# ISU-PAAL/DeepDFA

Hardware: NVIDIA H100
Metric: CFG graphs/sec (train step) (higher is better)
Workload: dtype f32 (GRU GEMMs: bf16x3 split operands, f32 accumulate)

## Files before the change

deepdfa_b200/csrc/gru_tc_fwd3.cu:

```cuda
#include <cuda_fp16.h>
#include <stdlib.h>

#include "tc_common.cuh"

namespace ddfa {
namespace tc3 {
using namespace tcc;

constexpr int kSlices = 4;
constexpr int kSliceCols = kD / kSlices;
constexpr int kRowsPerPart = 3 * kSliceCols;
constexpr int kWChunkBytes = kRowsPerPart * 128;
constexpr int kSliceWBytes = 8 * kWChunkBytes;
constexpr int kStageBytes = kImageTileBytes;
constexpr int kOffStage = kSliceWBytes;
constexpr int kOffBias = kOffStage + 2 * kStageBytes;
constexpr int kBiasSlice = 7 * kSliceCols;
constexpr int kOffBar = kOffBias + kBiasSlice * 4;
constexpr int kSmemAlloc = kOffBar + 5 * 8;
constexpr int kConsumerWarps = 8;
constexpr int kThreads = 32 * kConsumerWarps + 32;
constexpr size_t kPackedWBytes = (size_t)kSlices * kSliceWBytes;
constexpr size_t kPackedBytes = kPackedWBytes + (size_t)kSlices * kBiasSlice * 4;
static_assert(kSmemAlloc <= 232448, "shared memory budget");

__global__ void pack_kernel(const float *__restrict__ w_fold, const float *__restrict__ w_hh, const float *__restrict__ b_fold,
                            const float *__restrict__ b_ih, const float *__restrict__ b_hh, uint8_t *__restrict__ packed) {
  const int idx = blockIdx.x * blockDim.x + threadIdx.x;
  if (idx >= kSlices * 2 * kRowsPerPart * 16) return;
  const int u = idx % 16, n = (idx / 16) % kRowsPerPart, p = (idx / (16 * kRowsPerPart)) % 2, slice = idx / (32 * kRowsPerPart);
  const int kb = u >> 3, k0 = u * 8;
  const float *W = (p == 0 ? w_fold : w_hh) + (size_t)((n / kSliceCols) * kD + slice * kSliceCols + n % kSliceCols) * kD;
  float x[8];
#pragma unroll
  for (int i = 0; i < 8; ++i) x[i] = W[k0 + i];
  uint4 ph, pl;
  split8(x, ph, pl);
  uint8_t *base = packed + (size_t)slice * kSliceWBytes + sw128_offset(n, (u & 7) * 8);
  *reinterpret_cast<uint4 *>(base + ((p * 2 + 0) * 2 + kb) * kWChunkBytes) = ph;
  *reinterpret_cast<uint4 *>(base + ((p * 2 + 1) * 2 + kb) * kWChunkBytes) = pl;
  if (p == 0 && u == 0 && n < kSliceCols) {
    const int t = slice * kSliceCols + n;
    float *bias = reinterpret_cast<float *>(packed + kPackedWBytes) + slice * kBiasSlice;
    bias[0 * kSliceCols + n] = b_ih[2 * kD + t];
    bias[1 * kSliceCols + n] = b_ih[t] + b_hh[t];
    bias[2 * kSliceCols + n] = b_ih[kD + t] + b_hh[kD + t];
    bias[3 * kSliceCols + n] = b_hh[2 * kD + t];
    bias[4 * kSliceCols + n] = b_fold[2 * kD + t];
    bias[5 * kSliceCols + n] = b_fold[t];
    bias[6 * kSliceCols + n] = b_fold[kD + t];
  }
}

template <bool HIMG, int GATES>
__global__ void __launch_bounds__(kThreads, 1) gru_fwd3_kernel(const uint8_t *__restrict__ s_img, const uint8_t *__restrict__ h_img,
                                                               const float *__restrict__ h, const int32_t *__restrict__ indptr,
                                                               const uint8_t *__restrict__ packed, int32_t N,
                                                               float *__restrict__ h_out, uint8_t *__restrict__ h_out_img,
                                                               float *__restrict__ gates, uint2 *__restrict__ gates_packed, int hints) {
  extern __shared__ __align__(1024) uint8_t smem[];
  const uint32_t sbase = smem_u32(smem);
  if ((sbase & 1023u) != 0) __trap();
  const uint32_t bar0 = sbase + kOffBar;
  auto full = [&](int i) { return bar0 + 8u * i; };
  auto empty = [&](int i) { return bar0 + 8u * (2 + i); };
  const uint32_t w_full = bar0 + 32u;

  const int warp = threadIdx.x >> 5, lane = threadIdx.x & 31;
  const int slice = blockIdx.x % kSlices;
  const int group = blockIdx.x / kSlices, num_groups = gridDim.x / kSlices;
  const int num_tiles = (N + kTileM - 1) / kTileM;
  const int my_tiles = (num_tiles > group) ? (num_tiles - 1 - group) / num_groups + 1 : 0;

  if (threadIdx.x == 0) {
    for (int i = 0; i < 2; ++i) { mbar_init(full(i), 1); mbar_init(empty(i), kConsumerWarps); }
    mbar_init(w_full, 1);
    mbar_fence_init();
  }
  __syncthreads();
  const int tron = g_trace_on;
  if (threadIdx.x == 0) trace_stamp(tron, 0, 0);
  pdl_launch_dependents();

  if (warp == kConsumerWarps) {
    if (my_tiles > 0 && elect_one()) {
      mbar_arrive_expect_tx(w_full, kSliceWBytes);
      bulk_g2s(sbase, packed + (size_t)slice * kSliceWBytes, kSliceWBytes, w_full);
      pdl_wait();
      for (int k = 0; k < my_tiles; ++k) {
        const size_t toff = (size_t)(group + k * num_groups) * kImageTileBytes;
        for (int p = 0; p < 2; ++p) {
          if (k > 0) mbar_wait_bounded(empty(p), (k - 1) & 1);
          mbar_arrive_expect_tx(full(p), kStageBytes);
          bulk_g2s(sbase + kOffStage + p * kStageBytes, (p == 0 ? s_img : h_img) + toff, kStageBytes, full(p));
          trace_stamp(tron, k, 1 + p);
        }
      }
    }
    return;
  }

  float *sbias = reinterpret_cast<float *>(smem + kOffBias);
  for (int i = threadIdx.x; i < kBiasSlice; i += 32 * kConsumerWarps)
    sbias[i] = __ldcg(reinterpret_cast<const float *>(packed + kPackedWBytes) + slice * kBiasSlice + i);
  asm volatile("bar.sync 1, %0;" ::"n"(32 * kConsumerWarps) : "memory");
  pdl_wait();
  if (my_tiles == 0) return;
  const int wg = warp >> 2;
  const int row0 = wg * 64 + (warp & 3) * 16 + (lane >> 2);
  const int c4 = 2 * (lane & 3);
  const size_t plane = (size_t)N * kD;
  const uint64_t pol_gates = l2_policy((hints & 1) ? 1 : 0);
  const uint64_t pol_next = l2_policy((hints & 16) ? 2 : 0);
  mbar_wait_bounded(w_full, 0);
  const bool tr = (warp == 0 && lane == 0);

  for (int k = 0; k < my_tiles; ++k) {
    const int tile = group + k * num_groups;
    float acc_s[48], acc_h[48];
    if (tr) { trace_stamp(tron, k, 7); trace_stamp(tron, k, 3); }
    mbar_wait_bounded(full(0), k & 1);
    if (tr) trace_stamp(tron, k, 4);
    wgmma_fence();
#pragma unroll
    for (int p = 0; p < 2; ++p) {
      if (p == 1) {
        mbar_wait_bounded(full(1), k & 1);
        if (tr) trace_stamp(tron, k, 5);
      }
      const uint32_t a0 = sbase + kOffStage + p * kStageBytes + wg * 8192;
      const uint32_t w0 = sbase + p * 4 * kWChunkBytes;
#pragma unroll
      for (int kb = 0; kb < 2; ++kb) {
#pragma unroll
        for (int k4 = 0; k4 < 4; ++k4) {
          const uint64_t a_hi = gmma_desc(a0 + kb * kChunkBytes + k4 * 32), a_lo = gmma_desc(a0 + (2 + kb) * kChunkBytes + k4 * 32);
          const uint64_t b_hi = gmma_desc(w0 + kb * kWChunkBytes + k4 * 32), b_lo = gmma_desc(w0 + (2 + kb) * kWChunkBytes + k4 * 32);
          const uint32_t acc = (kb == 0 && k4 == 0) ? 0u : 1u;
          if (p == 0) {
            wgmma_n96<0, 0>(acc_s, a_hi, b_hi, acc);
            wgmma_n96<0, 0>(acc_s, a_hi, b_lo, 1u);
            wgmma_n96<0, 0>(acc_s, a_lo, b_hi, 1u);
          } else {
            wgmma_n96<0, 0>(acc_h, a_hi, b_hi, acc);
            wgmma_n96<0, 0>(acc_h, a_hi, b_lo, 1u);
            wgmma_n96<0, 0>(acc_h, a_lo, b_hi, 1u);
          }
        }
      }
      wgmma_commit();
    }
    float deg[2], hp[2][8];
#pragma unroll
    for (int hh = 0; hh < 2; ++hh) {
      const int64_t node = (int64_t)tile * kTileM + row0 + 8 * hh;
      const bool valid = node < N;
      deg[hh] = valid ? (float)(__ldcg(indptr + node + 1) - __ldcg(indptr + node)) : 0.f;
#pragma unroll
      for (int j = 0; j < 4; ++j) {
        const int gcol = slice * kSliceCols + 8 * j + c4;
        if constexpr (HIMG) {
          const uint32_t whi = __ldcg(reinterpret_cast<const uint32_t *>(h_img + image_offset(node, gcol, 0)));
          const uint32_t wlo = __ldcg(reinterpret_cast<const uint32_t *>(h_img + image_offset(node, gcol, 1)));
          hp[hh][2 * j] = __uint_as_float(whi << 16) + __uint_as_float(wlo << 16);
          hp[hh][2 * j + 1] = __uint_as_float(whi & 0xffff0000u) + __uint_as_float(wlo & 0xffff0000u);
        } else {
          const float2 v = valid ? __ldcg(reinterpret_cast<const float2 *>(h + node * kD + gcol)) : make_float2(0.f, 0.f);
          hp[hh][2 * j] = v.x;
          hp[hh][2 * j + 1] = v.y;
        }
      }
    }
    wgmma_wait<0>();
    wgmma_fence_regs(acc_s);
    wgmma_fence_regs(acc_h);
    if (tr) { trace_stamp(tron, k, 6); trace_stamp(tron, k, 8); }
    __syncwarp();
    if (lane == 0) { mbar_arrive(empty(0)); mbar_arrive(empty(1)); }
    if (tr) trace_stamp(tron, k, 9);

#pragma unroll
    for (int hh = 0; hh < 2; ++hh) {
      const int64_t node = (int64_t)tile * kTileM + row0 + 8 * hh;
      const bool valid = node < N;
#pragma unroll
      for (int j = 0; j < 4; ++j) {
        const int c = 8 * j + c4, gcol = slice * kSliceCols + c;
        float hn[2], rr[2], zz[2], nn[2], gg[2];
#pragma unroll
        for (int e = 0; e < 2; ++e) {
          const int i = 2 * hh + e;
          const float dg = deg[hh];
          const float gin = acc_s[4 * (8 + j) + i] + fmaf(dg, sbias[4 * kSliceCols + c + e], sbias[c + e]);
          const float r = fast_sigmoid(acc_s[4 * j + i] + acc_h[4 * j + i] + fmaf(dg, sbias[5 * kSliceCols + c + e], sbias[kSliceCols + c + e]));
          const float z = fast_sigmoid(acc_s[4 * (4 + j) + i] + acc_h[4 * (4 + j) + i] +
                                       fmaf(dg, sbias[6 * kSliceCols + c + e], sbias[2 * kSliceCols + c + e]));
          const float ghn = acc_h[4 * (8 + j) + i] + sbias[3 * kSliceCols + c + e];
          const float n = fast_tanh(fmaf(r, ghn, gin));
          hn[e] = valid ? fmaf(z, hp[hh][2 * j + e] - n, n) : 0.f;
          rr[e] = r; zz[e] = z; nn[e] = n; gg[e] = ghn;
        }
        const size_t off = (size_t)node * kD + gcol;
        if (valid && h_out != nullptr) st_f2_hint(h_out + off, make_float2(hn[0], hn[1]), pol_next);
        if constexpr (GATES == 2) {
          if (valid) {
            const uint2 g0 = pack_gates(rr[0], zz[0], nn[0], gg[0]), g1 = pack_gates(rr[1], zz[1], nn[1], gg[1]);
            st_u4_hint(gates_packed + off, make_uint4(g0.x, g0.y, g1.x, g1.y), pol_gates);
          }
        }
        if constexpr (GATES == 1) {
          if (valid) {
            st_f2_hint(gates + off, make_float2(rr[0], rr[1]), pol_gates);
            st_f2_hint(gates + plane + off, make_float2(zz[0], zz[1]), pol_gates);
            st_f2_hint(gates + 2 * plane + off, make_float2(nn[0], nn[1]), pol_gates);
            st_f2_hint(gates + 3 * plane + off, make_float2(gg[0], gg[1]), pol_gates);
          }
        }
        if (h_out_img != nullptr) {
          const uint32_t hw = bf16x2_bits(hn[0], hn[1]);
          const uint32_t lw = bf16x2_bits(hn[0] - __uint_as_float(hw << 16), hn[1] - __uint_as_float(hw & 0xffff0000u));
          st_u32_hint(h_out_img + image_offset(node, gcol, 0), hw, pol_next);
          st_u32_hint(h_out_img + image_offset(node, gcol, 1), lw, pol_next);
        }
      }
    }
    if (tr) trace_stamp(tron, k, 10);
  }
}

}

size_t gru_tc3_packed_bytes() { return tc3::kPackedBytes; }

int gru_tc3_prepare(const float *w_fold, const float *b_fold, const float *b_ih, const float *w_hh, const float *b_hh, void *packed,
                    cudaStream_t stream) {
  const int total = tc3::kSlices * 2 * tc3::kRowsPerPart * 16;
  tc3::pack_kernel<<<(total + 127) / 128, 128, 0, stream>>>(w_fold, w_hh, b_fold, b_ih, b_hh, static_cast<uint8_t *>(packed));
  DDFA_CHECK_LAUNCH("tc3::pack_kernel");
  chain_break();
  return DDFA_OK;
}

int gru_tc3_step_fwd(const void *s_img, const void *h_img, const float *h, const int32_t *indptr, int32_t N, float *h_out,
                     void *h_out_img, float *save_gates, void *save_gates_packed, const void *packed, cudaStream_t stream) {
  const int tiles = (N + tcc::kTileM - 1) / tcc::kTileM;
  int groups = kNumSMs / tc3::kSlices;
  if (groups > tiles) groups = tiles;
  if (save_gates && save_gates_packed) {
    set_error("tcgen05 engine (fwd): both gate formats requested");
    return DDFA_ERR_INVALID_ARG;
  }
  if ((h == nullptr && save_gates) ) {
    set_error("tcgen05 engine (fwd): fp32 gate planes go with the fp32 h operand (legacy form)");
    return DDFA_ERR_INVALID_ARG;
  }
  if (tiles == 0) return DDFA_OK;
#define DDFA_FWD3_LAUNCH(HIMG, GATES)                                                                                                     \
  do {                                                                                                                                   \
    DDFA_CUDA(cudaFuncSetAttribute(tc3::gru_fwd3_kernel<HIMG, GATES>, cudaFuncAttributeMaxDynamicSharedMemorySize, tc3::kSmemAlloc));     \
    DDFA_CUDA(launch_chain(2, tc3::gru_fwd3_kernel<HIMG, GATES>, dim3(groups * tc3::kSlices), dim3(tc3::kThreads), tc3::kSmemAlloc,        \
                           stream, static_cast<const uint8_t *>(s_img), static_cast<const uint8_t *>(h_img), h, indptr,                   \
                           static_cast<const uint8_t *>(packed), N, h_out, static_cast<uint8_t *>(h_out_img), save_gates,                \
                           static_cast<uint2 *>(save_gates_packed), l2_hints()));                                                        \
  } while (0)
  if (h) {
    if (save_gates) DDFA_FWD3_LAUNCH(false, 1);
    else if (save_gates_packed) DDFA_FWD3_LAUNCH(false, 2);
    else DDFA_FWD3_LAUNCH(false, 0);
  } else {
    if (save_gates_packed) DDFA_FWD3_LAUNCH(true, 2);
    else DDFA_FWD3_LAUNCH(true, 0);
  }
#undef DDFA_FWD3_LAUNCH
  DDFA_CHECK_LAUNCH("tc3::gru_fwd3_kernel");
  return DDFA_OK;
}

namespace tc3 {
__global__ void __launch_bounds__(256) to_image_kernel(const float *__restrict__ x, int32_t N, uint8_t *__restrict__ image) {
  const int64_t t = blockIdx.x * (int64_t)blockDim.x + threadIdx.x;
  const int64_t rows = ((int64_t)N + kTileM - 1) / kTileM * kTileM;
  if (t >= rows * 16) return;
  const int64_t node = t >> 4;
  const int col = (int)(t & 15) * 8;
  float v[8] = {0.f, 0.f, 0.f, 0.f, 0.f, 0.f, 0.f, 0.f};
  if (node < N) {
    const float4 a = ldg_nc_f4(x + node * kD + col), b = ldg_nc_f4(x + node * kD + col + 4);
    v[0] = a.x; v[1] = a.y; v[2] = a.z; v[3] = a.w; v[4] = b.x; v[5] = b.y; v[6] = b.z; v[7] = b.w;
  }
  uint4 ph, pl;
  split8(v, ph, pl);
  *reinterpret_cast<uint4 *>(image + image_offset(node, col, 0)) = ph;
  *reinterpret_cast<uint4 *>(image + image_offset(node, col, 1)) = pl;
}
}

size_t act_image_bytes(int64_t n) { return tcc::image_bytes(n); }

int act_to_image(const float *x, int32_t N, void *image, cudaStream_t stream) {
  const int64_t rows = ((int64_t)N + tcc::kTileM - 1) / tcc::kTileM * tcc::kTileM;
  const int64_t total = rows * 16;
  if (total == 0) return DDFA_OK;
  tc3::to_image_kernel<<<(unsigned)((total + 255) / 256), 256, 0, stream>>>(x, N, static_cast<uint8_t *>(image));
  DDFA_CHECK_LAUNCH("to_image_kernel");
  return DDFA_OK;
}

size_t gru_tc2_workspace_bytes() { return gru_tc3_packed_bytes(); }

int gru_tc2_prepare(const float *w_fold, const float *b_fold, const float *b_ih, const float *w_hh, const float *b_hh,
                    void *workspace, size_t workspace_bytes, cudaStream_t stream) {
  if (workspace == nullptr || workspace_bytes < gru_tc2_workspace_bytes()) {
    set_error("tcgen05 engine: workspace too small (%zu < %zu)", workspace_bytes, gru_tc2_workspace_bytes());
    return DDFA_ERR_WORKSPACE;
  }
  return gru_tc3_prepare(w_fold, b_fold, b_ih, w_hh, b_hh, workspace, stream);
}

int gru_tc2_step_fwd(const void *s_img, const void *h_img, const float *h, const int32_t *indptr, int32_t N, float *h_out,
                     void *h_out_img, float *save_gates, void *save_gates_packed, const void *workspace, size_t workspace_bytes,
                     cudaStream_t stream) {
  if (workspace == nullptr || workspace_bytes < gru_tc2_workspace_bytes()) {
    set_error("tcgen05 engine: workspace too small (%zu < %zu)", workspace_bytes, gru_tc2_workspace_bytes());
    return DDFA_ERR_WORKSPACE;
  }
  return gru_tc3_step_fwd(s_img, h_img, h, indptr, N, h_out, h_out_img, save_gates, save_gates_packed, workspace, stream);
}

int gru_tc3_trace_enable(int on) {
  DDFA_CUDA(cudaMemcpyToSymbol(tcc::g_trace_on, &on, sizeof(int)));
  return DDFA_OK;
}
int gru_tc3_trace_read(void *host, size_t bytes) {
  if (bytes > tcc::kTraceWords * sizeof(long long)) bytes = tcc::kTraceWords * sizeof(long long);
  DDFA_CUDA(cudaMemcpyFromSymbol(host, tcc::g_trace, bytes));
  return DDFA_OK;
}

}
```

Before: 115,200.

## Split stage barriers per warpgroup and ping-pong wgmma issue between warpgroups

Each stage load is split into per-warpgroup halves, each with its own full/empty mbarriers, so a warpgroup can start as soon as its own 64 rows have arrived. The two consumer warpgroups take turns issuing their wgmma sequences via named barriers (bar.sync/bar.arrive), so one warpgroup's GEMM can overlap the other's epilogue. It also interleaves the s and h GEMMs inside the k loop. The cost is more bulk copies (four chunk copies per half), extra barrier traffic, and serialized MMA issue, which could leave the tensor cores idle if the epilogues are short.

Result: no change. 115,500 (median of 6 runs) (+0.3%).

```diff
diff --git a/deepdfa_b200/csrc/gru_tc_fwd3.cu b/deepdfa_b200/csrc/gru_tc_fwd3.cu
--- a/deepdfa_b200/csrc/gru_tc_fwd3.cu
+++ b/deepdfa_b200/csrc/gru_tc_fwd3.cu
@@ -17,9 +17,12 @@
 constexpr int kOffBias = kOffStage + 2 * kStageBytes;
 constexpr int kBiasSlice = 7 * kSliceCols;
 constexpr int kOffBar = kOffBias + kBiasSlice * 4;
-constexpr int kSmemAlloc = kOffBar + 5 * 8;
+constexpr int kSmemAlloc = kOffBar + 9 * 8;
 constexpr int kConsumerWarps = 8;
 constexpr int kThreads = 32 * kConsumerWarps + 32;
+constexpr int kHalfRowsBytes = 64 * 128;
+constexpr int kHalfStageBytes = 4 * kHalfRowsBytes;
+constexpr int kTurn0 = 2, kTurn1 = 3;
 constexpr size_t kPackedWBytes = (size_t)kSlices * kSliceWBytes;
 constexpr size_t kPackedBytes = kPackedWBytes + (size_t)kSlices * kBiasSlice * 4;
 static_assert(kSmemAlloc <= 232448, "shared memory budget");
@@ -62,9 +65,9 @@
   const uint32_t sbase = smem_u32(smem);
   if ((sbase & 1023u) != 0) __trap();
   const uint32_t bar0 = sbase + kOffBar;
-  auto full = [&](int i) { return bar0 + 8u * i; };
-  auto empty = [&](int i) { return bar0 + 8u * (2 + i); };
-  const uint32_t w_full = bar0 + 32u;
+  auto full = [&](int p, int wg) { return bar0 + 8u * (2 * p + wg); };
+  auto empty = [&](int p, int wg) { return bar0 + 8u * (4 + 2 * p + wg); };
+  const uint32_t w_full = bar0 + 64u;
 
   const int warp = threadIdx.x >> 5, lane = threadIdx.x & 31;
   const int slice = blockIdx.x % kSlices;
@@ -73,7 +76,8 @@
   const int my_tiles = (num_tiles > group) ? (num_tiles - 1 - group) / num_groups + 1 : 0;
 
   if (threadIdx.x == 0) {
-    for (int i = 0; i < 2; ++i) { mbar_init(full(i), 1); mbar_init(empty(i), kConsumerWarps); }
+    for (int p = 0; p < 2; ++p)
+      for (int wg = 0; wg < 2; ++wg) { mbar_init(full(p, wg), 1); mbar_init(empty(p, wg), kConsumerWarps / 2); }
     mbar_init(w_full, 1);
     mbar_fence_init();
   }
@@ -89,11 +93,16 @@
       pdl_wait();
       for (int k = 0; k < my_tiles; ++k) {
         const size_t toff = (size_t)(group + k * num_groups) * kImageTileBytes;
-        for (int p = 0; p < 2; ++p) {
-          if (k > 0) mbar_wait_bounded(empty(p), (k - 1) & 1);
-          mbar_arrive_expect_tx(full(p), kStageBytes);
-          bulk_g2s(sbase + kOffStage + p * kStageBytes, (p == 0 ? s_img : h_img) + toff, kStageBytes, full(p));
-          trace_stamp(tron, k, 1 + p);
+        for (int wg = 0; wg < 2; ++wg) {
+          for (int p = 0; p < 2; ++p) {
+            if (k > 0) mbar_wait_bounded(empty(p, wg), (k - 1) & 1);
+            mbar_arrive_expect_tx(full(p, wg), kHalfStageBytes);
+            const uint32_t dst = sbase + kOffStage + p * kStageBytes + wg * kHalfRowsBytes;
+            const uint8_t *src = (p == 0 ? s_img : h_img) + toff + wg * kHalfRowsBytes;
+#pragma unroll
+            for (int c = 0; c < 4; ++c) bulk_g2s(dst + c * kChunkBytes, src + c * kChunkBytes, kHalfRowsBytes, full(p, wg));
+          }
+          trace_stamp(tron, k, 1 + wg);
         }
       }
     }
@@ -114,42 +123,48 @@
   const uint64_t pol_next = l2_policy((hints & 16) ? 2 : 0);
   mbar_wait_bounded(w_full, 0);
   const bool tr = (warp == 0 && lane == 0);
+  const bool tr1 = (warp == 4 && lane == 0);
+  auto wait_turn = [&]() {
+    if (wg == 0) asm volatile("bar.sync %0, %1;" ::"n"(kTurn0), "n"(32 * kConsumerWarps) : "memory");
+    else asm volatile("bar.sync %0, %1;" ::"n"(kTurn1), "n"(32 * kConsumerWarps) : "memory");
+  };
+  auto pass_turn = [&]() {
+    if (wg == 0) asm volatile("bar.arrive %0, %1;" ::"n"(kTurn1), "n"(32 * kConsumerWarps) : "memory");
+    else asm volatile("bar.arrive %0, %1;" ::"n"(kTurn0), "n"(32 * kConsumerWarps) : "memory");
+  };
 
   for (int k = 0; k < my_tiles; ++k) {
     const int tile = group + k * num_groups;
     float acc_s[48], acc_h[48];
-    if (tr) { trace_stamp(tron, k, 7); trace_stamp(tron, k, 3); }
-    mbar_wait_bounded(full(0), k & 1);
+    if (tr) trace_stamp(tron, k, 7);
+    if (wg == 1 || k > 0) wait_turn();
+    if (tr) trace_stamp(tron, k, 3);
+    mbar_wait_bounded(full(0, wg), k & 1);
     if (tr) trace_stamp(tron, k, 4);
+    mbar_wait_bounded(full(1, wg), k & 1);
+    if (tr) trace_stamp(tron, k, 5);
     wgmma_fence();
-#pragma unroll
-    for (int p = 0; p < 2; ++p) {
-      if (p == 1) {
-        mbar_wait_bounded(full(1), k & 1);
-        if (tr) trace_stamp(tron, k, 5);
+    const uint32_t a0 = sbase + kOffStage + wg * kHalfRowsBytes;
+#pragma unroll
+    for (int kb = 0; kb < 2; ++kb) {
+#pragma unroll
+      for (int k4 = 0; k4 < 4; ++k4) {
+        const uint32_t acc = (kb == 0 && k4 == 0) ? 0u : 1u;
+#pragma unroll
+        for (int p = 0; p < 2; ++p) {
+          const uint32_t ap = a0 + p * kStageBytes, wp = sbase + p * 4 * kWChunkBytes;
+          const uint64_t a_hi = gmma_desc(ap + kb * kChunkBytes + k4 * 32), a_lo = gmma_desc(ap + (2 + kb) * kChunkBytes + k4 * 32);
+          const uint64_t b_hi = gmma_desc(wp + kb * kWChunkBytes + k4 * 32), b_lo = gmma_desc(wp + (2 + kb) * kWChunkBytes + k4 * 32);
+          float(&d)[48] = p == 0 ? acc_s : acc_h;
+          wgmma_n96<0, 0>(d, a_hi, b_hi, acc);
+          wgmma_n96<0, 0>(d, a_hi, b_lo, 1u);
+          wgmma_n96<0, 0>(d, a_lo, b_hi, 1u);
+        }
       }
-      const uint32_t a0 = sbase + kOffStage + p * kStageBytes + wg * 8192;
-      const uint32_t w0 = sbase + p * 4 * kWChunkBytes;
-#pragma unroll
-      for (int kb = 0; kb < 2; ++kb) {
-#pragma unroll
-        for (int k4 = 0; k4 < 4; ++k4) {
-          const uint64_t a_hi = gmma_desc(a0 + kb * kChunkBytes + k4 * 32), a_lo = gmma_desc(a0 + (2 + kb) * kChunkBytes + k4 * 32);
-          const uint64_t b_hi = gmma_desc(w0 + kb * kWChunkBytes + k4 * 32), b_lo = gmma_desc(w0 + (2 + kb) * kWChunkBytes + k4 * 32);
-          const uint32_t acc = (kb == 0 && k4 == 0) ? 0u : 1u;
-          if (p == 0) {
-            wgmma_n96<0, 0>(acc_s, a_hi, b_hi, acc);
-            wgmma_n96<0, 0>(acc_s, a_hi, b_lo, 1u);
-            wgmma_n96<0, 0>(acc_s, a_lo, b_hi, 1u);
-          } else {
-            wgmma_n96<0, 0>(acc_h, a_hi, b_hi, acc);
-            wgmma_n96<0, 0>(acc_h, a_hi, b_lo, 1u);
-            wgmma_n96<0, 0>(acc_h, a_lo, b_hi, 1u);
-          }
-        }
-      }
-      wgmma_commit();
     }
+    wgmma_commit();
+    if (wg == 0 || k + 1 < my_tiles) pass_turn();
+    if (tr) trace_stamp(tron, k, 6);
     float deg[2], hp[2][8];
 #pragma unroll
     for (int hh = 0; hh < 2; ++hh) {
@@ -174,9 +189,10 @@
     wgmma_wait<0>();
     wgmma_fence_regs(acc_s);
     wgmma_fence_regs(acc_h);
-    if (tr) { trace_stamp(tron, k, 6); trace_stamp(tron, k, 8); }
+    if (tr) trace_stamp(tron, k, 8);
+    if (tr1) trace_stamp(tron, k, 11);
     __syncwarp();
-    if (lane == 0) { mbar_arrive(empty(0)); mbar_arrive(empty(1)); }
+    if (lane == 0) { mbar_arrive(empty(0, wg)); mbar_arrive(empty(1, wg)); }
     if (tr) trace_stamp(tron, k, 9);
 
 #pragma unroll
```
